# e4s2022/e4s

Measured on AMD Instinct MI355X. Metric: 1024^2 face-swap images/sec, higher is better.
Workload: dtype f32 operands as hi+lo bf16, 3 bf16 MFMAs per product, f32 accumulate (bf16x3) on the 3x3 convs whose launch fills the chip; exact f32 elsewhere; 1 GPU; E4S-core face swap at 1024^2 (2x Net3 encoder @256^2, style swap, 12 LocalMLPs, mask-guided StyleGAN2 generator K=13), BASELINE.json configs[3] shard: 8 swaps per GPU per step; per_gpu_batch=8, global_batch=8, out_size=1024, hip_graph=True, precision=as bf16x3 where the launch fills the chip (this batch), else exact fp32, parallelism=image-parallel x1

## Files before the change

### e4s_amd/csrc/conv_wino.hip

```cpp
#include "common.h"
#include <stdlib.h>
#include <type_traits>

int e4s_launch_wino1w(const e4s_conv_params& p, int ntn, int tx_n, int per_img, int ntiles, int grid, hipStream_t st);

namespace {

typedef __bf16 bf16x8 __attribute__((ext_vector_type(8)));
typedef __bf16 bf16x4 __attribute__((ext_vector_type(4)));

constexpr int NTHR = 512;
constexpr int TH = 16, TW = 16, NPAIR = TW / 2;
constexpr int VROWS = (TH + 2) * NPAIR;
constexpr int BN = 128, KC = 16, ROWB = 64;
constexpr int A_PLANE = VROWS * ROWB, A_BYTES = 4 * A_PLANE;
constexpr int B_PLANE = BN * ROWB, B_BYTES = 4 * B_PLANE;
#ifndef E4S_WINO_READS_FIRST
#define E4S_WINO_READS_FIRST 1
#endif
constexpr int WT_MIN_CHUNKS = 32;
constexpr int NITEMS = VROWS * 4;
constexpr int SMEM_WINO = 2 * A_BYTES + 2 * B_BYTES + 4 * BN * 2 * 8;

__device__ __forceinline__ int swz(int row, int g) { return row * ROWB + ((g ^ ((row >> 2) & 3)) << 4); }

__device__ __forceinline__ void split_store4(unsigned char* hi_dst, unsigned char* lo_dst, const f32x4 v) {
    const bf16x4 h = __builtin_convertvector(v, bf16x4);
    const f32x4 r = v - __builtin_convertvector(h, f32x4);
    const bf16x4 l = __builtin_convertvector(r, bf16x4);
    *reinterpret_cast<bf16x4*>(hi_dst) = h;
    *reinterpret_cast<bf16x4*>(lo_dst) = l;
}

__global__ void wino_weights_kernel(const float* __restrict__ w9, unsigned char* __restrict__ out, int Cout, int Cin) {
    const int64_t i = (int64_t)blockIdx.x * blockDim.x + threadIdx.x;
// ... 549 lines not shown
    cper = nchunk;
    if (tiles > 128 || nchunk < 4) return;
    int want = (int)((256 + tiles - 1) / tiles);
    if (want > nchunk / 2) want = nchunk / 2;
    if (want < 2) return;
    const int c = (nchunk + want - 1) / want, k = (nchunk + c - 1) / c;
    if (k < 2 || nchunk - (k - 1) * c < 2) return;
    ksplit = k;
    cper = c;
}

bool wino_covers(const e4s_conv_params& p) {
    return p.istride == 1 && p.ostride == 1 && p.ntaps == 9 && p.ncls == 1 && !p.labels && !p.rows && !p.in_scale && !p.out_scale &&
           !p.noise && p.y_cstride == 0 && p.Hi == p.Ho && p.Wi == p.Wo && p.Ha == p.Ho && p.Wa == p.Wo && p.Hi % TH == 0 &&
           p.Wi % TW == 0 && p.Cin % KC == 0 && p.Cin >= 2 * KC && p.Cout % BN == 0 && p.B > 0 &&
           (p.stats_ws == nullptr || p.stats_slots == (p.Hi / TH) * (p.Wi / TW));
}

}

extern "C" int64_t e4s_wino_weights_bytes(int Cout, int Cin) {
    if (Cout <= 0 || Cin <= 0 || Cin % KC) return -1;
    return (int64_t)3 * (Cin / KC) * 4 * Cout * ROWB * (Cout % 32 == 0 ? 2 : 1);
}

extern "C" int e4s_wino_weights_f32(const float* w9, void* out, int Cout, int Cin, void* stream) {
    if (!w9 || !out || Cout <= 0 || Cin <= 0 || Cin % KC) return (int)hipErrorInvalidValue;
    const int64_t total = (int64_t)3 * Cout * Cin;
    hipLaunchKernelGGL(wino_weights_kernel, dim3((unsigned)((total + 255) / 256)), dim3(256), 0, as_stream(stream), w9,
                       reinterpret_cast<unsigned char*>(out), Cout, Cin);
    E4S_CHECK_LAUNCH();
    return 0;
}

extern "C" int e4s_conv_wino_covers(const e4s_conv_params* p) { return p && wino_covers(*p) ? 1 : 0; }

extern "C" int64_t e4s_conv_wino_ws_floats(const e4s_conv_params* pp) {
    if (!pp || !wino_covers(*pp)) return 0;
    const e4s_conv_params& p = *pp;
    int ksplit, cper;
    wino_split(p, (int64_t)p.B * (p.Hi / TH) * (p.Wi / TW) * (p.Cout / BN), ksplit, cper);
    return ksplit > 1 ? (int64_t)ksplit * p.B * p.Ho * p.Wo * p.Cout : 0;
}

extern "C" int e4s_conv_wino_bf16x3_f32(const e4s_conv_params* pp, void* stream) {
    if (!pp) return (int)hipErrorInvalidValue;
    const e4s_conv_params& p = *pp;
    if (!p.x || !p.w || !p.y || !wino_covers(p)) return (int)hipErrorInvalidValue;
    if (p.act == 2 && !p.slope) return (int)hipErrorInvalidValue;
    const int tx_n = p.Wi / TW, per_img = (p.Hi / TH) * tx_n, ntn = p.Cout / BN;
// ... 10 lines not shown
    {
        static std::atomic<uint64_t> mv[11];
        const char* ev = getenv("E4S_WINO_VAR");
        const int var = ev ? atoi(ev) : 0;
        const void* fn = nullptr;
#define WV(V) case V: fn = (const void*)conv_wino_kernel<0, V>; if ((e = e4s_ensure_dyn_smem(fn, SMEM_WINO, mv[V]))) return e; \
              hipLaunchKernelGGL((conv_wino_kernel<0, V>), dim3((unsigned)grid), dim3(NTHR), SMEM_WINO, as_stream(stream), p, ntn, tx_n, per_img, (int)tiles, ksplit, cper); \
              E4S_CHECK_LAUNCH(); return 0;
        switch (p.in_stats ? 0 : var) {
            WV(1) WV(2) WV(3) WV(4) WV(5) WV(6) WV(7) WV(8) WV(9) WV(10)
            default: break;
        }
#undef WV
    }
#endif
    {
        const char* e1 = getenv("E4S_WINO_1W");
        const bool want = e1 ? atoi(e1) != 0 : (p.Cin / KC >= 8 && p.Cout % 32 == 0);
        if (ksplit == 1 && want) return e4s_launch_wino1w(p, ntn, tx_n, per_img, (int)tiles, (int)grid, as_stream(stream));
    }
    const char* wt_env = getenv("E4S_WINO_WT");
    const bool wt = wt_env ? atoi(wt_env) != 0 : (p.Cin / KC) / (ksplit > 0 ? ksplit : 1) >= WT_MIN_CHUNKS;
    if (wt) {
        static std::atomic<uint64_t> w0{0}, w2{0};
        if (p.in_stats) {
            if (p.Cin > 1024) return (int)hipErrorInvalidValue;
            if ((e = e4s_ensure_dyn_smem((const void*)conv_wino_kernel<2, 0, 1>, SMEM_WINO + 16384, w2))) return e;
            hipLaunchKernelGGL((conv_wino_kernel<2, 0, 1>), dim3((unsigned)grid), dim3(NTHR), SMEM_WINO + p.Cin * 16, as_stream(stream), p, ntn,
                               tx_n, per_img, (int)tiles, ksplit, cper);
        } else {
            if ((e = e4s_ensure_dyn_smem((const void*)conv_wino_kernel<0, 0, 1>, SMEM_WINO, w0))) return e;
            hipLaunchKernelGGL((conv_wino_kernel<0, 0, 1>), dim3((unsigned)grid), dim3(NTHR), SMEM_WINO, as_stream(stream), p, ntn, tx_n, per_img,
                               (int)tiles, ksplit, cper);
        }
    } else if (p.in_stats) {
// ... 14 lines not shown
```

### e4s_amd/csrc/conv_wino1w.hip

```cpp
#include "common.h"
#include <stdlib.h>
#include <type_traits>

namespace {

typedef __bf16 bf16x8 __attribute__((ext_vector_type(8)));
typedef __bf16 bf16x2 __attribute__((ext_vector_type(2)));
typedef float f32x2 __attribute__((ext_vector_type(2)));
typedef unsigned u32x2 __attribute__((ext_vector_type(2)));

constexpr int NTHR = 256;
constexpr int TH = 16, TW = 16, NPAIR = TW / 2;
constexpr int VROWS = (TH + 2) * NPAIR;
constexpr int BN = 128, KC = 16, ROWB = 64;
constexpr int A_PLANE = VROWS * ROWB, A_BYTES = 4 * A_PLANE;
constexpr int OFF_IN = 2 * A_BYTES;
constexpr int SMEM_1W = OFF_IN;
#ifndef E4S_WINO_BPF
#define E4S_WINO_BPF 1
#endif
constexpr int BPF = E4S_WINO_BPF;
static_assert(BPF == 1 || BPF == 2, "B prefetch distance");

__device__ __forceinline__ int swz(int row, int g) { return row * ROWB + ((g ^ ((row >> 2) & 3)) << 4); }

__device__ __forceinline__ void lds_barrier() {
    __builtin_amdgcn_fence(__ATOMIC_RELEASE, "workgroup", "local");
    __builtin_amdgcn_s_barrier();
    __builtin_amdgcn_fence(__ATOMIC_ACQUIRE, "workgroup", "local");
}

struct WTile {
    int n0, tb, ty0, tx0, slot;
};

struct AF { bf16x8 h[4], l[4]; };
struct BF { bf16x8 h, l; };

template <int XF>
__device__ __forceinline__ void pair_split(const float a0, const float b0, const float a1, const float b1, const float m0, const float m1,
                                           const float sg, const float r0, const float r1, unsigned& hi, unsigned& lo) {
    float v0 = __builtin_fmaf(sg, b0 - m0, a0 - m0), v1 = __builtin_fmaf(sg, b1 - m1, a1 - m1);
    if (XF == 2) {
        v0 *= r0;
        v1 *= r1;
    }
    hi = __builtin_bit_cast(unsigned, __builtin_convertvector(f32x2{v0, v1}, bf16x2));
    const float e0 = v0 - __builtin_bit_cast(float, hi << 16), e1 = v1 - __builtin_bit_cast(float, hi & 0xffff0000u);
    lo = __builtin_bit_cast(unsigned, __builtin_convertvector(f32x2{e0, e1}, bf16x2));
}

template <int XF, int VAR = 0>
__global__ __launch_bounds__(NTHR) __attribute__((amdgpu_waves_per_eu(1, 1)))
void conv_wino1w_kernel(const e4s_conv_params p, const int ntn, const int tx_n, const int per_img, const int ntiles) {
    extern __shared__ __attribute__((aligned(16))) unsigned char smem[];
    unsigned char* sA = smem;
    float* s_in = reinterpret_cast<float*>(smem + OFF_IN);

    const int tid = threadIdx.x;
    const int lane = tid & 63, wave = __builtin_amdgcn_readfirstlane(tid >> 6);
    const int li = lane & 31, kh = lane >> 5;
    const int wn = wave;
    const int G = gridDim.x;
    const int first = xcd_remap(blockIdx.x, G);
    const int mtiles = ntiles / ntn;
    const int nchunk = p.Cin / KC;
    const unsigned char* ub = reinterpret_cast<const unsigned char*>(p.w);
    auto decode = [&](int t) -> WTile {
        WTile w;
        const int nt = t / mtiles, mt = t - nt * mtiles;
        w.n0 = nt * BN;
        w.tb = mt / per_img;
        w.slot = mt - w.tb * per_img;
        const int tyb = w.slot / tx_n;
        w.ty0 = tyb * TH;
        w.tx0 = (w.slot - tyb * tx_n) * TW;
        return w;
    };

    const int cq = tid & 3;
    auto rel_of = [&](int v) -> int { return (((v >> 3) - 1) * p.Wi + 2 * (v & 7) - 1) * p.Cin + cq * 4; };
    auto flg_of = [&](int v) -> unsigned { return ((v >> 3) == 0 ? 1u : 0u) | ((v >> 3) == 17 ? 2u : 0u) | ((v & 7) == 0 ? 4u : 0u) | ((v & 7) == 7 ? 8u : 0u); };
    auto dst_of = [&](int v) -> int { return swz(v, cq >> 1) + (cq & 1) * 8; };
    const int vA = tid >> 2, vB = 64 + (tid >> 2), vQ = 128 + (lane >> 2);
    const int relA = rel_of(vA), relB = rel_of(vB), relQ = rel_of(vQ);
    const unsigned flgA = flg_of(vA), flgB = flg_of(vB), flgQ = flg_of(vQ);
    const int dstA = dst_of(vA), dstB = dst_of(vB), dstQ = dst_of(vQ) + wave * A_PLANE;
    const int qa = wave == 0 ? 0 : (wave == 2 ? 2 : 1), qb = wave == 0 ? 2 : (wave == 1 ? 2 : (wave == 2 ? 1 : 3));
    const float qsg = wave == 1 ? 1.f : -1.f;
    auto edge_of = [&](const WTile& T) -> unsigned {
        return (T.ty0 == 0 ? 1u : 0u) | (T.ty0 + TH == p.Hi ? 2u : 0u) | (T.tx0 == 0 ? 4u : 0u) | (T.tx0 + TW == p.Wi ? 8u : 0u);
    };
    auto xbase_of = [&](const WTile& T, int chunk) -> const float* {
        return p.x + (size_t)T.tb * p.Hi * p.Wi * p.Cin + ((size_t)T.ty0 * p.Wi + T.tx0) * p.Cin + chunk * KC;
    };
    auto load_px = [&](const float* xb, int rel, unsigned bad, int i, bool& ok) -> f32x4 {
        ok = !((bad & 3u) || (i == 0 && (bad & 4u)) || (i == 3 && (bad & 8u)));
        return *reinterpret_cast<const f32x4*>(xb + (ok ? rel + i * p.Cin : cq * 4));
    };
// ... 36 lines not shown
        }
        hi = __builtin_bit_cast(unsigned, __builtin_convertvector(f32x2{v[0], v[1]}, bf16x2));
        const float e0 = v[0] - __builtin_bit_cast(float, hi << 16), e1 = v[1] - __builtin_bit_cast(float, hi & 0xffff0000u);
        lo = __builtin_bit_cast(unsigned, __builtin_convertvector(f32x2{e0, e1}, bf16x2));
    };
    auto load_stats = [&](const WTile& T, int par) {
        if (XF == 2) {
            const float* st = p.in_stats + (size_t)T.tb * p.Cin * 2;
            for (int i = tid * 4; i < p.Cin * 2; i += NTHR * 4)
                *reinterpret_cast<f32x4*>(s_in + par * p.Cin * 2 + i) = *reinterpret_cast<const f32x4*>(st + i);
        }
    };

    const unsigned char* uf = ub + (size_t)3 * nchunk * 4 * p.Cout * ROWB;
    auto uf_src = [&](int ky, int chunk, int ps, int n0) -> const unsigned char* {
        return uf + ((((size_t)ky * nchunk + chunk) * 4 + ps) * (p.Cout / 32) + (n0 / 32 + wn)) * 2048 + lane * 16;
    };
    if (first >= ntiles) return;
    WTile cur = decode(first);
    int t_next = first + G;
    bool has_next = t_next < ntiles;
    WTile nxt = decode(has_next ? t_next : first);

    Item I;
    f32x4 Qa, Qb;
    bool Qoka = true, Qokb = true;
    I.okmask = 0;
    load_stats(cur, 0);
    if (XF == 2) __syncthreads();
    {
        const float* xb0 = xbase_of(cur, 0);
// ... 12 lines not shown
                item_pair(I0, mu, rs, ps, 0, h[0], l[0]);
                item_pair(I0, mu, rs, ps, 1, h[1], l[1]);
                const int a = ps * A_PLANE + dst_of(v);
                *reinterpret_cast<u32x2*>(sA + a) = u32x2{h[0], h[1]};
                *reinterpret_cast<u32x2*>(sA + (a ^ 32)) = u32x2{l[0], l[1]};
            }
        }
        const float* xb1 = xbase_of(cur, 1);
#pragma unroll
        for (int i = 0; i < 4; ++i) item_load_part(I, xb1, relA, flgA & edge, i);
        Qa = load_px(xb1, relQ, flgQ & edge, qa, Qoka);
        Qb = load_px(xb1, relQ, flgQ & edge, qb, Qokb);
    }
    __syncthreads();

    int aoff[4][3];
#pragma unroll
    for (int tm = 0; tm < 4; ++tm)
#pragma unroll
        for (int ky = 0; ky < 3; ++ky) aoff[tm][ky] = swz(tm * 32 + li + 8 * ky, kh);

    f32x16 acc[4][4];
    AF Af[2];
    BF Bf[BPF == 1 ? 1 : 3][4];
    auto ldA = [&](AF& F, const unsigned char* Abuf, int ps, int ky, int part) {
        const unsigned char* a = Abuf + ps * A_PLANE;
        const int tm = part >> 1;
        if (part & 1) F.l[tm] = *reinterpret_cast<const bf16x8*>(a + (aoff[tm][ky] ^ 32));
        else F.h[tm] = *reinterpret_cast<const bf16x8*>(a + aoff[tm][ky]);
    };
#pragma unroll
    for (int part = 0; part < 8; ++part) ldA(Af[0], sA, 0, 0, part);
#pragma unroll
    for (int ps = 0; ps < 4; ++ps) {
        const unsigned char* b = uf_src(0, 0, ps, cur.n0);
        Bf[0][ps].h = *reinterpret_cast<const bf16x8*>(b);
        Bf[0][ps].l = *reinterpret_cast<const bf16x8*>(b + 1024);
        if (BPF == 2) {
            const unsigned char* b1 = uf_src(1, 0, ps, cur.n0);
            Bf[1][ps].h = *reinterpret_cast<const bf16x8*>(b1);
            Bf[1][ps].l = *reinterpret_cast<const bf16x8*>(b1 + 1024);
        }
    }

    unsigned sg = 0, cg = 0;
    int par = 0;
    f32x4 mu = {0.f, 0.f, 0.f, 0.f}, rs = {1.f, 1.f, 1.f, 1.f};
    unsigned hh[2], ll[2];
    for (;;) {
        if (has_next) load_stats(nxt, par ^ 1);
        const unsigned edge_c = edge_of(cur), edge_n = edge_of(nxt);
#pragma unroll
        for (int ps = 0; ps < 4; ++ps)
#pragma unroll
            for (int tm = 0; tm < 4; ++tm)
#pragma unroll
                for (int r = 0; r < 16; ++r) acc[ps][tm][r] = 0.f;

        for (int chunk = 0; chunk < nchunk; ++chunk) {
            const bool in_tile = chunk + 1 < nchunk;
            const WTile& Tn = in_tile ? cur : nxt;
            const int c_n = in_tile ? chunk + 1 : 0;
            const int par_n = in_tile ? par : par ^ 1;
            const unsigned char* Ab = sA + (cg & 1) * A_BYTES;
            unsigned char* An = sA + ((cg + 1) & 1) * A_BYTES;
            const bool in2 = chunk + 2 < nchunk;
            const WTile& T2 = in2 ? cur : nxt;
            const int c_2 = in2 ? chunk + 2 : (chunk + 2 - nchunk);
            const unsigned edge_nn = in_tile ? edge_c : edge_n, edge_2 = in2 ? edge_c : edge_n;
            const float* xb_n = xbase_of(Tn, c_n);
            const float* xb_2 = xbase_of(T2, c_2);
            auto stage = [&](auto ts_c) {
                constexpr int ts = decltype(ts_c)::value;
                constexpr int ky1 = (ts + BPF) % 3;
                const int ch1 = ts + BPF < 3 ? chunk : c_n, n01 = ts + BPF < 3 ? cur.n0 : Tn.n0;
                constexpr int bs_cur = BPF == 1 ? 0 : ts, bs_ld = BPF == 1 ? 0 : (ts + 2) % 3;
#pragma unroll
                for (int ps = 0; ps < 4; ++ps) {
                    AF& Ac = Af[ps & 1];
                    AF& Ax = Af[(ps + 1) & 1];
                    const BF Bc = Bf[bs_cur][ps];
                    const unsigned char* nA = ps < 3 ? Ab : (ts < 2 ? Ab : An);
                    const int nps = (ps + 1) & 3, nky = ps < 3 ? ts : (ts + 1) % 3;
                    const unsigned char* nb = uf_src(ky1, ch1, ps, n01);
#pragma unroll
                    for (int k = 0; k < 12; ++k) {
                        const int prod = k >> 2, tm = k & 3;
                        acc[ps][tm] = prod == 0 ? __builtin_amdgcn_mfma_f32_32x32x16_bf16(Ac.h[tm], Bc.l, acc[ps][tm], 0, 0, 0)
                                    : prod == 1 ? __builtin_amdgcn_mfma_f32_32x32x16_bf16(Ac.l[tm], Bc.h, acc[ps][tm], 0, 0, 0)
                                                : __builtin_amdgcn_mfma_f32_32x32x16_bf16(Ac.h[tm], Bc.h, acc[ps][tm], 0, 0, 0);
                        if (VAR == 4) {
                            if (k == 0) Ax = Ac;
                        } else if (k < 8) ldA(Ax, nA, nps, nky, k);
                        if (VAR == 0 || VAR == 2) {
                            if (k == 8) Bf[bs_ld][ps].l = *reinterpret_cast<const bf16x8*>(nb + 1024);
                            if (k == 11) Bf[bs_ld][ps].h = *reinterpret_cast<const bf16x8*>(nb);
                        }
                        if (ps >= 2 && (VAR == 0 || VAR == 1)) {
                            const int n = (ps - 2) * 12 + k;
                            if (ts < 2 && n < 16) {
                                const int q = n >> 2, piece = n & 3;
                                if (n == 0) {
                                    stats_of(mu, rs, c_n, par_n);
                                    item_fill(I, mu);
                                }
                                if (piece == 0) item_pair(I, mu, rs, q, 0, hh[0], ll[0]);
                                if (piece == 1) item_pair(I, mu, rs, q, 1, hh[1], ll[1]);
                                const int a = q * A_PLANE + (ts == 0 ? dstA : dstB);
                                if (piece == 2) *reinterpret_cast<u32x2*>(An + a) = u32x2{hh[0], hh[1]};
                                if (piece == 3) *reinterpret_cast<u32x2*>(An + (a ^ 32)) = u32x2{ll[0], ll[1]};
                            }
                            if (ts == 0 && n >= 16 && n < 20) {
                                const f32x4 fill = XF == 2 ? mu : f32x4{0.f, 0.f, 0.f, 0.f};
                                const f32x4 da = Qoka ? Qa : fill, db = Qokb ? Qb : fill;
                                const bool nrm = XF == 2 && wave == 1;
                                if (n == 16) pair_split<XF>(da[0], db[0], da[1], db[1], nrm ? mu[0] : 0.f, nrm ? mu[1] : 0.f, qsg, rs[0], rs[1], hh[0], ll[0]);
                                if (n == 17) pair_split<XF>(da[2], db[2], da[3], db[3], nrm ? mu[2] : 0.f, nrm ? mu[3] : 0.f, qsg, rs[2], rs[3], hh[1], ll[1]);
                                if (n == 18) *reinterpret_cast<u32x2*>(An + dstQ) = u32x2{hh[0], hh[1]};
                                if (n == 19) *reinterpret_cast<u32x2*>(An + (dstQ ^ 32)) = u32x2{ll[0], ll[1]};
                            }
                            if (ts == 0 && n >= 20) item_load_part(I, xb_n, relB, flgB & edge_nn, n - 20);
                            if (ts == 2 && n >= 16 && n < 20) item_load_part(I, xb_2, relA, flgA & edge_2, n - 16);
                            if (ts == 2 && n == 20) Qa = load_px(xb_2, relQ, flgQ & edge_2, qa, Qoka);
                            if (ts == 2 && n == 21) Qb = load_px(xb_2, relQ, flgQ & edge_2, qb, Qokb);
                        }
                        __builtin_amdgcn_sched_barrier(0);
                    }
                    if (ps == 1 && VAR != 4) {
                        lds_barrier();
                        __builtin_amdgcn_sched_barrier(0);
                    }
                }
                ++sg;
            };
            stage(std::integral_constant<int, 0>{});
            stage(std::integral_constant<int, 1>{});
            stage(std::integral_constant<int, 2>{});
            ++cg;
        }

        {
            const float gain = (p.act == 1) ? p.gain : 1.f;
            const bool do_act = p.act != 0;
            const bool stats = p.stats_ws != nullptr;
            float* yb = p.y + (size_t)cur.tb * p.Ho * p.Wo * p.Cout;
            const int co = cur.n0 + wn * 32 + li;
            const float bsv = p.bias ? p.bias[co] : 0.f;
            const float slp = (p.act == 2) ? p.slope[co] : p.alpha;
            double st_s = 0.0, st_q = 0.0;
#pragma unroll
            for (int tm = 0; tm < 4; ++tm) {
#pragma unroll
                for (int g = 0; g < 4; ++g) {
                    float y0[4], y1[4];
#pragma unroll
                    for (int i = 0; i < 4; ++i) {
                        const int r = 4 * g + i;
                        const float m0 = acc[0][tm][r], m1 = acc[1][tm][r], m2 = acc[2][tm][r], m3 = acc[3][tm][r];
                        float a = (m0 + m1) + m2 + bsv;
                        float b = (m1 - m2) - m3 + bsv;
                        if (do_act) {
                            a = (a > 0.f ? a : a * slp) * gain;
                            b = (b > 0.f ? b : b * slp) * gain;
                        }
                        y0[i] = a;
                        y1[i] = b;
                        if (stats) {
                            st_s += (double)a + (double)b;
                            st_q += (double)a * (double)a + (double)b * (double)b;
                        }
                    }
                    quad_transpose4(y0[0], y0[1], y0[2], y0[3], li);
                    quad_transpose4(y1[0], y1[1], y1[2], y1[3], li);
// ... 11 lines not shown
                    double* slot = p.stats_ws + (((size_t)cur.tb * p.Cout + co) * p.stats_slots + cur.slot) * 2;
                    slot[0] = st_s;
                    slot[1] = st_q;
                }
            }
        }
        if (!has_next) break;
        cur = nxt;
        par ^= 1;
        t_next += G;
        has_next = t_next < ntiles;
        if (has_next) nxt = decode(t_next);
    }
}

}

int e4s_launch_wino1w(const e4s_conv_params& p, int ntn, int tx_n, int per_img, int ntiles, int grid, hipStream_t st) {
    static std::atomic<uint64_t> m0{0}, m2{0};
    int e;
#ifdef E4S_ABLATIONS
    {
        const char* ev = getenv("E4S_WINO_1W_VAR");
        const int var = ev ? atoi(ev) : 0;
        const void* fn = nullptr;
#define WV(V) case V: fn = (const void*)conv_wino1w_kernel<0, V>; if ((e = (int)hipFuncSetAttribute(fn, hipFuncAttributeMaxDynamicSharedMemorySize, SMEM_1W))) return e; \
              hipLaunchKernelGGL((conv_wino1w_kernel<0, V>), dim3((unsigned)grid), dim3(NTHR), SMEM_1W, st, p, ntn, tx_n, per_img, ntiles); \
              E4S_CHECK_LAUNCH(); return 0;
        switch (p.in_stats ? 0 : var) {
            WV(1) WV(2) WV(3) WV(4)
            default: break;
        }
#undef WV
    }
#endif
    if (p.in_stats) {
        if (p.Cin > 1024) return (int)hipErrorInvalidValue;
        if ((e = e4s_ensure_dyn_smem((const void*)conv_wino1w_kernel<2>, SMEM_1W + 16384, m2))) return e;
        hipLaunchKernelGGL(conv_wino1w_kernel<2>, dim3((unsigned)grid), dim3(NTHR), SMEM_1W + p.Cin * 16, st, p, ntn, tx_n, per_img, ntiles);
    } else {
        if ((e = e4s_ensure_dyn_smem((const void*)conv_wino1w_kernel<0>, SMEM_1W, m0))) return e;
        hipLaunchKernelGGL(conv_wino1w_kernel<0>, dim3((unsigned)grid), dim3(NTHR), SMEM_1W, st, p, ntn, tx_n, per_img, ntiles);
    }
    E4S_CHECK_LAUNCH();
    return 0;
}
```

### e4s_amd/csrc/ops.hip

```cpp
#include "common.h"

namespace {

__device__ __forceinline__ float bias_act_one(float x, float ref, int code, float alpha, float scale) {
    float y;
    switch (code) {
        case 12: case 32: y = 0.f; break;
        case 30: y = (x > 0.f) ? x : x * alpha; break;
        case 31: y = (ref > 0.f) ? x : x * alpha; break;
        default: y = x; break;
    }
    return y * scale;
}

__global__ void fused_bias_act_v4(const f32x4* __restrict__ x, const float* __restrict__ b,
                                  const f32x4* __restrict__ ref, f32x4* __restrict__ y, int64_t n4,
                                  int step_b, int size_b, int code, float alpha, float scale) {
    const int64_t stride = (int64_t)gridDim.x * blockDim.x;
    for (int64_t i = (int64_t)blockIdx.x * blockDim.x + threadIdx.x; i < n4; i += stride) {
        f32x4 v = x[i];
        if (b) {
            const float bv = b[((i * 4) / step_b) % size_b];
            v += bv;
        }
// ... 75 lines not shown
        if (oy >= out_h || ox >= out_w) continue;
        const int my = oy * down_y - pad_y0, mx = ox * down_x - pad_x0;
        const int iy_first = floordiv(my + up_y - 1, up_y), ix_first = floordiv(mx + up_x - 1, up_x);
        float acc = 0.f;
        for (int iy = iy_first, jy = iy_first * up_y - my; jy < kh; ++iy, jy += up_y) {
            const float* row = sx + (iy - in_y0) * tin_w;
            for (int ix = ix_first, jx = ix_first * up_x - mx; jx < kw; ++ix, jx += up_x)
                acc += row[ix - in_x0] * sk[jy * kw + jx];
        }
        y[(((int64_t)mj * out_h + oy) * out_w + ox) * minor + mi] = acc;
    }
}

}

extern "C" int e4s_abi_version(void) { return 15; }
extern "C" const char* e4s_build_arch(void) { return "gfx950"; }

extern "C" int e4s_fused_bias_act_f32(const float* x, const float* b, const float* ref, float* y, int64_t n,
                                      int step_b, int size_b, int act, int grad, float alpha, float scale,
                                      void* stream) {
    if (n <= 0) return 0;
    const int code = act * 10 + grad;
    if (code == 31 && !ref) return (int)hipErrorInvalidValue;
    if (b && (step_b <= 0 || size_b <= 0)) return (int)hipErrorInvalidValue;
    const bool vec = (n % 4 == 0) && (!b || step_b % 4 == 0) &&
                     ((reinterpret_cast<uintptr_t>(x) | reinterpret_cast<uintptr_t>(y) |
                       reinterpret_cast<uintptr_t>(ref)) % 16 == 0);
    const int block = 256;
    if (vec) {
        const int64_t n4 = n / 4;
// ... 135 lines not shown
```

### e4s_amd/kernels.py

```python
import contextlib
import ctypes
import math
import os
import threading

import torch

from . import lib
from .lib import ConvBwdParams, ConvParams, ConvWgradParams, c_p, call, fptr, ptr, stream

BM = 128
PRECISION = os.environ.get("E4S_PRECISION", "auto")
if PRECISION not in ("f32", "bf16x3", "auto"):
    raise RuntimeError(f"E4S_PRECISION must be f32, bf16x3 or auto, got {PRECISION!r}")
BF16X3_MIN_BLOCKS = int(os.environ.get("E4S_BF16X3_MIN_BLOCKS", "128"))
LRELU_GAIN = math.sqrt(2.0)


def _f32(t):
    if t.dtype != torch.float32:
        raise RuntimeError(f"expected float32 tensor, got {t.dtype}")
    return t.contiguous()


# ... 376 lines not shown

def split16_bf16x2(w, out=None):
    w = _f32(w)
    out = _into(out, split16_shape(w.shape), w.device)
    cout, cin = w.shape[-2], w.shape[-1]
    rows = w.numel() // (cout * cin)
    if lib.load().e4s_split16_bytes(rows, cout, cin) != out.numel() * 4:
        raise RuntimeError("split16_bf16x2: buffer size")
    call("e4s_split16_bf16x2_f32", fptr(w), ptr(out), rows, cout, cin, stream())
    return out


REGION_1W = os.environ.get("E4S_REGION_1W", "1") != "0"
LAST_REGION_PATH = 0
WINO = os.environ.get("E4S_WINO", "1") == "1"


def wino_eligible(b, h, w, cin, cout, in_stats=False):
    if not WINO or PRECISION == "f32":
        return False
    if h % 16 or w % 16 or cin % 16 or cin < 32 or cout % 128:
        return False
    if in_stats and cin > 1024:
        return False
    if PRECISION == "bf16x3":
        return True
    tiles = b * (h // 16) * (w // 16) * (cout // 128)
    if tiles >= BF16X3_MIN_BLOCKS:
        return True
    nchunk = cin // 16
# ... 19 lines not shown
    y = torch.empty(b, h, w, cout, device=x.device, dtype=torch.float32)
    p = ConvParams()
    p.x, p.w, p.y = fptr(x), ptr(u), fptr(y)
    p.rows = p.tiles = p.meta = None
    p.B, p.Ha, p.Wa, p.Hi, p.Wi, p.Ho, p.Wo, p.Cin, p.Cout = b, h, w, h, w, h, w, cin, cout
    p.istride, p.ostride, p.ntaps, p.ncls, p.groups_per_batch = 1, 1, 9, 1, 1
    p.bias, p.slope = fptr(bias), fptr(slope)
    p.act, p.alpha, p.gain = act, alpha, gain
    p.in_stats = fptr(in_stats)
    fused = None
    if want_stats and act != 0:
        raise RuntimeError("conv_wino: output statistics are those of the raw conv output (act = 0)")
    nws = lib.load().e4s_conv_wino_ws_floats(ctypes.byref(p))
    skws = torch.empty(nws, device=x.device, dtype=torch.float32) if nws else None
    p.splitk_ws = fptr(skws)
    if want_stats and not nws:
        slots = (h // 16) * (w // 16)
        fused = torch.empty(b * cout * slots * 2, device=x.device, dtype=torch.float64)
        p.stats_ws, p.stats_slots = ptr(fused), slots
    call("e4s_conv_wino_bf16x3_f32", ctypes.byref(p), stream())
    if fused is None:
        if not want_stats:
            return y
        stats, pooled = instnorm_stats(y, want_pooled=True)
        return y, (stats, se_gate(pooled, se[0], se[1]) if se is not None else pooled)
    stats = torch.empty(b, cout, 2, device=x.device, dtype=torch.float32)
    pooled = torch.empty(b, cout, device=x.device, dtype=torch.float32)
    if se is not None:
        call("e4s_instnorm_finalize_se_f32", ptr(fused), fptr(stats), fptr(se[0]), fptr(se[1]), fptr(pooled), b, h * w, cout,
             se[0].shape[0], p.stats_slots, 1e-5, stream())
    else:
        call("e4s_instnorm_finalize_f32", ptr(fused), fptr(stats), fptr(pooled), b, h * w, cout, p.stats_slots, 1e-5, stream())
# ... 898 lines not shown
```

### e4s_amd/lib.py

```python
import ctypes
import os

import torch

_HERE = os.path.dirname(os.path.abspath(__file__))
LIB_PATH = os.environ.get("E4S_LIB_PATH") or os.path.join(_HERE, "libe4s_hip.so")
ABI_VERSION = 15

c_p = ctypes.c_void_p
c_i = ctypes.c_int
c_l = ctypes.c_int64
c_f = ctypes.c_float
c_d = ctypes.c_double


STYLE_GRAD_MAX_JOBS = 32


class StyleGradJob(ctypes.Structure):
    _fields_ = [
        ("ds_raw", c_p), ("dd_d", c_p), ("d", c_p), ("s", c_p), ("wsq", c_p), ("dws", c_p), ("w3", c_p), ("wmod", c_p), ("ds_total", c_p),
        ("conv_scale", c_f), ("mod_scale", c_f), ("G", c_i), ("Cin", c_i), ("Cout", c_i), ("slot", c_i), ("masked", c_i),
    ]

# ... 91 lines not shown
    "e4s_torgb_finish_f32": [c_p, c_p, c_p, c_p, c_p, c_i, c_i, c_i, c_p],
    "e4s_rowdot_multi_f32": [c_p, c_i, c_p, c_p, c_i, c_i, c_i, c_p],
    "e4s_ema_f32": [c_p, c_p, c_l, c_d, c_p],
    "e4s_adam_step_dev_f32": [c_p, c_p, c_p, c_p, c_l, c_d, c_p, c_d, c_d, c_d, c_d, c_p, c_p],
    "e4s_advance_i64": [c_p, c_l, c_p],
    "e4s_conv_smallcin_col2im_f32": [c_p, c_p] + [c_i] * 10 + [c_p],
    "e4s_region_scale_f32": [c_p, c_p, c_p, c_i, c_i, c_i, c_p, c_i, c_i, c_i, c_i, c_i, c_p],
    "e4s_col2im_region_nsplit": [c_i, c_i, c_i, c_i],
    "e4s_col2im_region_f32": [c_p, c_p, c_p, c_p, c_i, c_i, c_i, c_p, c_p, c_p, c_i, c_i, c_i, c_i, c_i, c_p],
    "e4s_act_bwd_demod_nsplit": [c_i, c_i, c_i, c_i],
    "e4s_act_bwd_demod_f32": [c_p, c_p, c_p, c_p, c_p, c_l, c_p, c_f, c_f, c_p, c_i, c_i, c_i, c_p, c_p, c_i, c_i, c_i, c_i, c_p],
    "e4s_pixel_unshuffle2_f32": [c_p, c_p, c_i, c_i, c_i, c_i, c_p],
    "e4s_wino_weights_bytes": [c_i, c_i],
    "e4s_wino_weights_f32": [c_p, c_p, c_i, c_i, c_p],
    "e4s_conv_wino_covers": [c_p],
    "e4s_conv_wino_ws_floats": [c_p],
    "e4s_conv_wino_bf16x3_f32": [c_p, c_p],
    "e4s_adam_multi_dev_f32": [c_i, c_p, c_p, c_p, c_p, c_p, c_p, c_d, c_p, c_d, c_d, c_d, c_d, c_p],
    "e4s_ema_multi_f32": [c_i, c_p, c_p, c_p, c_d, c_p],
    "e4s_torgb_bwd_x_f32": [c_p, c_p, c_p, c_i, c_i, c_i, c_p, c_i, c_i, c_i, c_i, c_i, c_p],
    "e4s_shift_scale_f32": [c_p, c_p, c_p, c_i, c_i, c_i, c_p] + [c_i] * 12 + [c_p],
    "e4s_torgb_f32": [c_p, c_p, c_p, c_p, c_p, c_p, c_i, c_i, c_i, c_p, c_i, c_i, c_i, c_i, c_p],
    "e4s_mask_mul_add_f32": [c_p, c_p, c_p] + [c_i] * 10 + [c_p],
    "e4s_noise_bias_act_nhwc_f32": [c_p, c_p, c_p, c_l, c_p, c_p, c_i, c_i, c_i, c_f, c_f, c_p],
    "e4s_nchw_to_nhwc_f32": [c_p, c_p, c_i, c_i, c_i, c_i, c_p],
    "e4s_nhwc_to_nchw_f32": [c_p, c_p, c_i, c_i, c_i, c_i, c_p],
    "e4s_const_input_f32": [c_p, c_p, c_i, c_i, c_i, c_i, c_p],
    "e4s_resize_bilinear_f32": [c_p, c_p] + [c_i] * 6 + [c_p],
    "e4s_conv3x3_small_f32": [c_p, c_p, c_p] + [c_i] * 5 + [c_p],
    "e4s_conv3x3_stem_f32": [c_p, c_p, c_p, c_p] + [c_i] * 5 + [c_p],
# ... 112 lines not shown
```

### include/e4s_hip.h

```cpp
#ifndef E4S_HIP_H
#define E4S_HIP_H
#include <stdint.h>

#ifdef __cplusplus
extern "C" {
#endif

int e4s_abi_version(void);
const char* e4s_build_arch(void);


int e4s_fused_bias_act_f32(const float* x, const float* b, const float* ref, float* y, int64_t n,
                           int step_b, int size_b, int act, int grad, float alpha, float scale,
                           void* stream);

int e4s_upfirdn2d_f32(const float* x, const float* k, float* y, int major, int in_h, int in_w, int minor,
                      int kh, int kw, int up_x, int up_y, int down_x, int down_y,
                      int pad_x0, int pad_x1, int pad_y0, int pad_y1, void* stream);

int e4s_channel_sum_f32(const float* g, float* out, int64_t n, int step_b, int size_b, void* stream);


int e4s_rowdot_f32(const float* in, int64_t in_stride, const float* M, const float* bias, float* out,
                   int G, int O, int K, int mode, float scale, void* stream);
// ... 189 lines not shown
int64_t e4s_colsum_ws_floats(int64_t rows, int C);
int e4s_scale_dot_f32(float* u, const float* x, const float* s, float* ds, float* ws, int B, int64_t hw, int C, void* stream);
int64_t e4s_scale_dot_ws_floats(int B, int64_t hw, int C);
int e4s_adam_step_f32(float* p, const float* grad, float* m, float* v, int64_t n, double lr, double beta1, double beta2,
                      double eps, double weight_decay, int step, void* stream);
int e4s_adam_step_dev_f32(float* p, const float* grad, float* m, float* v, int64_t n, double lr, const double* lr_dev, double beta1,
                          double beta2, double eps, double weight_decay, const int64_t* step, void* stream);
int e4s_advance_i64(int64_t* steps, int64_t n, void* stream);
int e4s_adam_multi_dev_f32(int count, float* const* p, const float* const* grad, float* const* m, float* const* v, const int64_t* n,
                           const int64_t* const* step, double lr, const double* lr_dev, double beta1, double beta2, double eps,
                           double weight_decay, void* stream);
int e4s_ema_multi_f32(int count, float* const* dst, const float* const* src, const int64_t* n, double decay, void* stream);
int64_t e4s_wino_weights_bytes(int Cout, int Cin);
int e4s_wino_weights_f32(const float* w9, void* out, int Cout, int Cin, void* stream);
int e4s_conv_wino_covers(const e4s_conv_params* p);
int64_t e4s_conv_wino_ws_floats(const e4s_conv_params* p);
int e4s_conv_wino_bf16x3_f32(const e4s_conv_params* p, void* stream);
int e4s_subpixel_weights_f32(const float* w, void* out, int Cout, int Cin, void* stream);
int e4s_upconv_bf16x3_f32(const e4s_conv_params* p, const float* k4, void* stream);

int e4s_conv_c32_bf16x3_f32(const e4s_conv_params* p, const float* rgb_ws, float* rgb_partial, void* stream);
int e4s_torgb_finish_f32(const float* partial, const float* bias, const float* skip, const float* k4, float* out, int B, int H,
                         int W, void* stream);

int e4s_mask_to_u8(const float* mask, uint8_t* out, int B, int H, int W, int Hm, int Wm, void* stream);
int e4s_erode_u8(const uint8_t* src, uint8_t* dst, int B, int H, int W, int radius, int border_value, void* stream);
int e4s_gaussian_blur_u8(const uint8_t* src, uint8_t* dst, int B, int H, int W, int ksize, const int* taps_fixed8, void* stream);
int e4s_alpha_composite_u8(const uint8_t* face, const uint8_t* target, const uint8_t* alpha, uint8_t* out, int B, int H, int W,
                           void* stream);
int e4s_pyrdown_u8(const uint8_t* src, uint8_t* dst, int B, int H, int W, int C, void* stream);
// ... 94 lines not shown
```

Baseline: 491.2 images/s.

## Add wide-N 8x16 tile variant to single-wave Winograd bf16x3 conv kernel

Templates the single-wave Winograd conv kernel on a tile shape. When Cout is a multiple of 256 (the default), the new variant uses 8-row spatial tiles with 256 output channels per block, so each wave holds two 32-column B fragments and two A row-tiles instead of one B and four A. This shifts reuse from the A operand toward the weights and changes how B loads are scheduled, and adds a stats-slot layout tied to the tile height, which the Python side now queries. Risks include higher register pressure from two B fragments, fewer tiles per image when filling the GPU, and weight prefetch being disabled for the wide path (BP=1).

```diff
diff --git a/e4s_amd/csrc/conv_wino.hip b/e4s_amd/csrc/conv_wino.hip
--- a/e4s_amd/csrc/conv_wino.hip
+++ b/e4s_amd/csrc/conv_wino.hip
@@ -2,7 +2,7 @@
 #include <stdlib.h>
 #include <type_traits>
 
-int e4s_launch_wino1w(const e4s_conv_params& p, int ntn, int tx_n, int per_img, int ntiles, int grid, hipStream_t st);
+int e4s_launch_wino1w(const e4s_conv_params& p, int wide, int ntn, int tx_n, int per_img, int ntiles, int grid, hipStream_t st);
 
 namespace {
 
@@ -19,6 +19,7 @@
 #define E4S_WINO_READS_FIRST 1
 #endif
 constexpr int WT_MIN_CHUNKS = 32;
+constexpr int TH_WIDE = 8, BN_WIDE = 256;
 constexpr int NITEMS = VROWS * 4;
 constexpr int SMEM_WINO = 2 * A_BYTES + 2 * B_BYTES + 4 * BN * 2 * 8;
 
@@ -598,7 +599,18 @@
     return p.istride == 1 && p.ostride == 1 && p.ntaps == 9 && p.ncls == 1 && !p.labels && !p.rows && !p.in_scale && !p.out_scale &&
            !p.noise && p.y_cstride == 0 && p.Hi == p.Ho && p.Wi == p.Wo && p.Ha == p.Ho && p.Wa == p.Wo && p.Hi % TH == 0 &&
            p.Wi % TW == 0 && p.Cin % KC == 0 && p.Cin >= 2 * KC && p.Cout % BN == 0 && p.B > 0 &&
-           (p.stats_ws == nullptr || p.stats_slots == (p.Hi / TH) * (p.Wi / TW));
+           (p.stats_ws == nullptr || p.stats_slots == (p.Hi / TH) * (p.Wi / TW) ||
+            (p.Cout % BN_WIDE == 0 && p.stats_slots == (p.Hi / TH_WIDE) * (p.Wi / TW)));
+}
+
+int wino_path(const e4s_conv_params& p, int ksplit) {
+    const char* e1 = getenv("E4S_WINO_1W");
+    const bool want = e1 ? atoi(e1) != 0 : (p.Cin / KC >= 8 && p.Cout % 32 == 0);
+    if (ksplit != 1 || !want) return 1;
+    if (p.Cout % BN_WIDE) return 2;
+    const char* et = getenv("E4S_WINO_1W_TILE");
+    const bool wide = et ? atoi(et) != 0 : true;
+    return wide ? 3 : 2;
 }
 
 }
@@ -618,6 +630,13 @@
 }
 
 extern "C" int e4s_conv_wino_covers(const e4s_conv_params* p) { return p && wino_covers(*p) ? 1 : 0; }
+
+extern "C" int e4s_conv_wino_path(const e4s_conv_params* pp) {
+    if (!pp || !wino_covers(*pp)) return 0;
+    int ksplit, cper;
+    wino_split(*pp, (int64_t)pp->B * (pp->Hi / TH) * (pp->Wi / TW) * (pp->Cout / BN), ksplit, cper);
+    return wino_path(*pp, ksplit);
+}
 
 extern "C" int64_t e4s_conv_wino_ws_floats(const e4s_conv_params* pp) {
     if (!pp || !wino_covers(*pp)) return 0;
@@ -658,11 +677,14 @@
 #undef WV
     }
 #endif
-    {
-        const char* e1 = getenv("E4S_WINO_1W");
-        const bool want = e1 ? atoi(e1) != 0 : (p.Cin / KC >= 8 && p.Cout % 32 == 0);
-        if (ksplit == 1 && want) return e4s_launch_wino1w(p, ntn, tx_n, per_img, (int)tiles, (int)grid, as_stream(stream));
+    const int path = wino_path(p, ksplit);
+    if (path >= 2) {
+        const bool wide = path == 3;
+        const int pi = wide ? (p.Hi / TH_WIDE) * tx_n : per_img;
+        if (p.stats_ws && p.stats_slots != pi) return (int)hipErrorInvalidValue;
+        return e4s_launch_wino1w(p, wide ? 1 : 0, wide ? p.Cout / BN_WIDE : ntn, tx_n, pi, (int)tiles, (int)grid, as_stream(stream));
     }
+    if (p.stats_ws && p.stats_slots != per_img) return (int)hipErrorInvalidValue;
     const char* wt_env = getenv("E4S_WINO_WT");
     const bool wt = wt_env ? atoi(wt_env) != 0 : (p.Cin / KC) / (ksplit > 0 ? ksplit : 1) >= WT_MIN_CHUNKS;
     if (wt) {
diff --git a/e4s_amd/csrc/conv_wino1w.hip b/e4s_amd/csrc/conv_wino1w.hip
--- a/e4s_amd/csrc/conv_wino1w.hip
+++ b/e4s_amd/csrc/conv_wino1w.hip
@@ -10,12 +10,19 @@
 typedef unsigned u32x2 __attribute__((ext_vector_type(2)));
 
 constexpr int NTHR = 256;
-constexpr int TH = 16, TW = 16, NPAIR = TW / 2;
-constexpr int VROWS = (TH + 2) * NPAIR;
-constexpr int BN = 128, KC = 16, ROWB = 64;
-constexpr int A_PLANE = VROWS * ROWB, A_BYTES = 4 * A_PLANE;
-constexpr int OFF_IN = 2 * A_BYTES;
-constexpr int SMEM_1W = OFF_IN;
+constexpr int TW = 16, NPAIR = TW / 2;
+constexpr int KC = 16, ROWB = 64;
+template <int W>
+struct Tile {
+    static constexpr int TH = W ? 8 : 16;
+    static constexpr int VROWS = (TH + 2) * NPAIR;
+    static constexpr int NTM = TH / 4, NCB = W ? 2 : 1;
+    static constexpr int BN = 4 * 32 * NCB;
+    static constexpr int A_PLANE = VROWS * ROWB, A_BYTES = 4 * A_PLANE;
+    static constexpr int VQ0 = VROWS - 16;
+    static constexpr int OFF_IN = 2 * A_BYTES;
+    static constexpr int SMEM = OFF_IN;
+};
 #ifndef E4S_WINO_BPF
 #define E4S_WINO_BPF 1
 #endif
@@ -34,8 +41,10 @@
     int n0, tb, ty0, tx0, slot;
 };
 
-struct AF { bf16x8 h[4], l[4]; };
-struct BF { bf16x8 h, l; };
+template <int NTM>
+struct AFt { bf16x8 h[NTM], l[NTM]; };
+template <int NCB>
+struct BFt { bf16x8 h[NCB], l[NCB]; };
 
 template <int XF>
 __device__ __forceinline__ void pair_split(const float a0, const float b0, const float a1, const float b1, const float m0, const float m1,
@@ -50,12 +59,17 @@
     lo = __builtin_bit_cast(unsigned, __builtin_convertvector(f32x2{e0, e1}, bf16x2));
 }
 
-template <int XF, int VAR = 0>
+template <int XF, int VAR = 0, int W = 0>
 __global__ __launch_bounds__(NTHR) __attribute__((amdgpu_waves_per_eu(1, 1)))
 void conv_wino1w_kernel(const e4s_conv_params p, const int ntn, const int tx_n, const int per_img, const int ntiles) {
+    using C = Tile<W>;
+    constexpr int TH = C::TH, VROWS = C::VROWS, BN = C::BN, A_PLANE = C::A_PLANE, A_BYTES = C::A_BYTES, NTM = C::NTM, NCB = C::NCB;
+    constexpr int BP = W ? 1 : BPF;
+    using AF = AFt<NTM>;
+    using BF = BFt<NCB>;
     extern __shared__ __attribute__((aligned(16))) unsigned char smem[];
     unsigned char* sA = smem;
-    float* s_in = reinterpret_cast<float*>(smem + OFF_IN);
+    float* s_in = reinterpret_cast<float*>(smem + C::OFF_IN);
 
     const int tid = threadIdx.x;
     const int lane = tid & 63, wave = __builtin_amdgcn_readfirstlane(tid >> 6);
@@ -80,9 +94,9 @@
 
     const int cq = tid & 3;
     auto rel_of = [&](int v) -> int { return (((v >> 3) - 1) * p.Wi + 2 * (v & 7) - 1) * p.Cin + cq * 4; };
-    auto flg_of = [&](int v) -> unsigned { return ((v >> 3) == 0 ? 1u : 0u) | ((v >> 3) == 17 ? 2u : 0u) | ((v & 7) == 0 ? 4u : 0u) | ((v & 7) == 7 ? 8u : 0u); };
+    auto flg_of = [&](int v) -> unsigned { return ((v >> 3) == 0 ? 1u : 0u) | ((v >> 3) == TH + 1 ? 2u : 0u) | ((v & 7) == 0 ? 4u : 0u) | ((v & 7) == 7 ? 8u : 0u); };
     auto dst_of = [&](int v) -> int { return swz(v, cq >> 1) + (cq & 1) * 8; };
-    const int vA = tid >> 2, vB = 64 + (tid >> 2), vQ = 128 + (lane >> 2);
+    const int vA = tid >> 2, vB = 64 + (tid >> 2), vQ = C::VQ0 + (lane >> 2);
     const int relA = rel_of(vA), relB = rel_of(vB), relQ = rel_of(vQ);
     const unsigned flgA = flg_of(vA), flgB = flg_of(vB), flgQ = flg_of(vQ);
     const int dstA = dst_of(vA), dstB = dst_of(vB), dstQ = dst_of(vQ) + wave * A_PLANE;
@@ -149,7 +163,12 @@
 
     const unsigned char* uf = ub + (size_t)3 * nchunk * 4 * p.Cout * ROWB;
     auto uf_src = [&](int ky, int chunk, int ps, int n0) -> const unsigned char* {
-        return uf + ((((size_t)ky * nchunk + chunk) * 4 + ps) * (p.Cout / 32) + (n0 / 32 + wn)) * 2048 + lane * 16;
+        return uf + ((((size_t)ky * nchunk + chunk) * 4 + ps) * (p.Cout / 32) + (n0 / 32 + wn * NCB)) * 2048 + lane * 16;
+    };
+    auto ldB = [&](BF& F, const unsigned char* b, int part) {
+        const int cb = part >> 1;
+        if (part & 1) F.l[cb] = *reinterpret_cast<const bf16x8*>(b + cb * 2048 + 1024);
+        else F.h[cb] = *reinterpret_cast<const bf16x8*>(b + cb * 2048);
     };
     if (first >= ntiles) return;
     WTile cur = decode(first);
@@ -192,15 +211,15 @@
     }
     __syncthreads();
 
-    int aoff[4][3];
-#pragma unroll
-    for (int tm = 0; tm < 4; ++tm)
+    int aoff[NTM][3];
+#pragma unroll
+    for (int tm = 0; tm < NTM; ++tm)
 #pragma unroll
         for (int ky = 0; ky < 3; ++ky) aoff[tm][ky] = swz(tm * 32 + li + 8 * ky, kh);
 
-    f32x16 acc[4][4];
+    f32x16 acc[4][NCB][NTM];
     AF Af[2];
-    BF Bf[BPF == 1 ? 1 : 3][4];
+    BF Bf[BP == 1 ? 1 : 3][4];
     auto ldA = [&](AF& F, const unsigned char* Abuf, int ps, int ky, int part) {
         const unsigned char* a = Abuf + ps * A_PLANE;
         const int tm = part >> 1;
@@ -208,16 +227,13 @@
         else F.h[tm] = *reinterpret_cast<const bf16x8*>(a + aoff[tm][ky]);
     };
 #pragma unroll
-    for (int part = 0; part < 8; ++part) ldA(Af[0], sA, 0, 0, part);
+    for (int part = 0; part < 2 * NTM; ++part) ldA(Af[0], sA, 0, 0, part);
 #pragma unroll
     for (int ps = 0; ps < 4; ++ps) {
-        const unsigned char* b = uf_src(0, 0, ps, cur.n0);
-        Bf[0][ps].h = *reinterpret_cast<const bf16x8*>(b);
-        Bf[0][ps].l = *reinterpret_cast<const bf16x8*>(b + 1024);
-        if (BPF == 2) {
-            const unsigned char* b1 = uf_src(1, 0, ps, cur.n0);
-            Bf[1][ps].h = *reinterpret_cast<const bf16x8*>(b1);
-            Bf[1][ps].l = *reinterpret_cast<const bf16x8*>(b1 + 1024);
+#pragma unroll
+        for (int part = 0; part < 2 * NCB; ++part) {
+            ldB(Bf[0][ps], uf_src(0, 0, ps, cur.n0), part);
+            if (BP == 2) ldB(Bf[1][ps], uf_src(1, 0, ps, cur.n0), part);
         }
     }
 
@@ -231,9 +247,11 @@
 #pragma unroll
         for (int ps = 0; ps < 4; ++ps)
 #pragma unroll
-            for (int tm = 0; tm < 4; ++tm)
-#pragma unroll
-                for (int r = 0; r < 16; ++r) acc[ps][tm][r] = 0.f;
+            for (int cb = 0; cb < NCB; ++cb)
+#pragma unroll
+                for (int tm = 0; tm < NTM; ++tm)
+#pragma unroll
+                    for (int r = 0; r < 16; ++r) acc[ps][cb][tm][r] = 0.f;
 
         for (int chunk = 0; chunk < nchunk; ++chunk) {
             const bool in_tile = chunk + 1 < nchunk;
@@ -250,9 +268,9 @@
             const float* xb_2 = xbase_of(T2, c_2);
             auto stage = [&](auto ts_c) {
                 constexpr int ts = decltype(ts_c)::value;
-                constexpr int ky1 = (ts + BPF) % 3;
-                const int ch1 = ts + BPF < 3 ? chunk : c_n, n01 = ts + BPF < 3 ? cur.n0 : Tn.n0;
-                constexpr int bs_cur = BPF == 1 ? 0 : ts, bs_ld = BPF == 1 ? 0 : (ts + 2) % 3;
+                constexpr int ky1 = (ts + BP) % 3;
+                const int ch1 = ts + BP < 3 ? chunk : c_n, n01 = ts + BP < 3 ? cur.n0 : Tn.n0;
+                constexpr int bs_cur = BP == 1 ? 0 : ts, bs_ld = BP == 1 ? 0 : (ts + 2) % 3;
 #pragma unroll
                 for (int ps = 0; ps < 4; ++ps) {
                     AF& Ac = Af[ps & 1];
@@ -263,20 +281,27 @@
                     const unsigned char* nb = uf_src(ky1, ch1, ps, n01);
 #pragma unroll
                     for (int k = 0; k < 12; ++k) {
-                        const int prod = k >> 2, tm = k & 3;
-                        acc[ps][tm] = prod == 0 ? __builtin_amdgcn_mfma_f32_32x32x16_bf16(Ac.h[tm], Bc.l, acc[ps][tm], 0, 0, 0)
-                                    : prod == 1 ? __builtin_amdgcn_mfma_f32_32x32x16_bf16(Ac.l[tm], Bc.h, acc[ps][tm], 0, 0, 0)
-                                                : __builtin_amdgcn_mfma_f32_32x32x16_bf16(Ac.h[tm], Bc.h, acc[ps][tm], 0, 0, 0);
+                        const int prod = k >> 2, tm = W ? (k & 1) : (k & 3), cb = W ? ((k >> 1) & 1) : 0;
+                        acc[ps][cb][tm] = prod == 0 ? __builtin_amdgcn_mfma_f32_32x32x16_bf16(Ac.h[tm], Bc.l[cb], acc[ps][cb][tm], 0, 0, 0)
+                                        : prod == 1 ? __builtin_amdgcn_mfma_f32_32x32x16_bf16(Ac.l[tm], Bc.h[cb], acc[ps][cb][tm], 0, 0, 0)
+                                                    : __builtin_amdgcn_mfma_f32_32x32x16_bf16(Ac.h[tm], Bc.h[cb], acc[ps][cb][tm], 0, 0, 0);
                         if (VAR == 4) {
                             if (k == 0) Ax = Ac;
-                        } else if (k < 8) ldA(Ax, nA, nps, nky, k);
+                        } else if (k < 2 * NTM) ldA(Ax, nA, nps, nky, k);
                         if (VAR == 0 || VAR == 2) {
-                            if (k == 8) Bf[bs_ld][ps].l = *reinterpret_cast<const bf16x8*>(nb + 1024);
-                            if (k == 11) Bf[bs_ld][ps].h = *reinterpret_cast<const bf16x8*>(nb);
+                            if (W) {
+                                if (k == 4) ldB(Bf[bs_ld][ps], nb, 1);
+                                if (k == 5) ldB(Bf[bs_ld][ps], nb, 3);
+                                if (k == 10) ldB(Bf[bs_ld][ps], nb, 0);
+                                if (k == 11) ldB(Bf[bs_ld][ps], nb, 2);
+                            } else {
+                                if (k == 8) ldB(Bf[bs_ld][ps], nb, 1);
+                                if (k == 11) ldB(Bf[bs_ld][ps], nb, 0);
+                            }
                         }
                         if (ps >= 2 && (VAR == 0 || VAR == 1)) {
                             const int n = (ps - 2) * 12 + k;
-                            if (ts < 2 && n < 16) {
+                            if (ts < (W ? 1 : 2) && n < 16) {
                                 const int q = n >> 2, piece = n & 3;
                                 if (n == 0) {
                                     stats_of(mu, rs, c_n, par_n);
@@ -297,7 +322,7 @@
                                 if (n == 18) *reinterpret_cast<u32x2*>(An + dstQ) = u32x2{hh[0], hh[1]};
                                 if (n == 19) *reinterpret_cast<u32x2*>(An + (dstQ ^ 32)) = u32x2{ll[0], ll[1]};
                             }
-                            if (ts == 0 && n >= 20) item_load_part(I, xb_n, relB, flgB & edge_nn, n - 20);
+                            if (!W && ts == 0 && n >= 20) item_load_part(I, xb_n, relB, flgB & edge_nn, n - 20);
                             if (ts == 2 && n >= 16 && n < 20) item_load_part(I, xb_2, relA, flgA & edge_2, n - 16);
                             if (ts == 2 && n == 20) Qa = load_px(xb_2, relQ, flgQ & edge_2, qa, Qoka);
                             if (ts == 2 && n == 21) Qb = load_px(xb_2, relQ, flgQ & edge_2, qb, Qokb);
@@ -317,24 +342,25 @@
             ++cg;
         }
 
-        {
+#pragma unroll
+        for (int cb = 0; cb < NCB; ++cb) {
             const float gain = (p.act == 1) ? p.gain : 1.f;
             const bool do_act = p.act != 0;
             const bool stats = p.stats_ws != nullptr;
             float* yb = p.y + (size_t)cur.tb * p.Ho * p.Wo * p.Cout;
-            const int co = cur.n0 + wn * 32 + li;
+            const int co = cur.n0 + (wn * NCB + cb) * 32 + li;
             const float bsv = p.bias ? p.bias[co] : 0.f;
             const float slp = (p.act == 2) ? p.slope[co] : p.alpha;
             double st_s = 0.0, st_q = 0.0;
 #pragma unroll
-            for (int tm = 0; tm < 4; ++tm) {
+            for (int tm = 0; tm < NTM; ++tm) {
 #pragma unroll
                 for (int g = 0; g < 4; ++g) {
                     float y0[4], y1[4];
 #pragma unroll
                     for (int i = 0; i < 4; ++i) {
                         const int r = 4 * g + i;
-                        const float m0 = acc[0][tm][r], m1 = acc[1][tm][r], m2 = acc[2][tm][r], m3 = acc[3][tm][r];
+                        const float m0 = acc[0][cb][tm][r], m1 = acc[1][cb][tm][r], m2 = acc[2][cb][tm][r], m3 = acc[3][cb][tm][r];
                         float a = (m0 + m1) + m2 + bsv;
                         float b = (m1 - m2) - m3 + bsv;
                         if (do_act) {
@@ -376,19 +402,26 @@
     }
 }
 
-}
-
-int e4s_launch_wino1w(const e4s_conv_params& p, int ntn, int tx_n, int per_img, int ntiles, int grid, hipStream_t st) {
-    static std::atomic<uint64_t> m0{0}, m2{0};
+template <int XF, int VAR, int W>
+int launch_1w(const e4s_conv_params& p, int ntn, int tx_n, int per_img, int ntiles, int grid, hipStream_t st) {
+    static std::atomic<uint64_t> done{0};
+    const int stat_bytes = XF == 2 ? p.Cin * 16 : 0;
     int e;
+    if ((e = e4s_ensure_dyn_smem((const void*)conv_wino1w_kernel<XF, VAR, W>, Tile<W>::SMEM + (XF == 2 ? 16384 : 0), done))) return e;
+    hipLaunchKernelGGL((conv_wino1w_kernel<XF, VAR, W>), dim3((unsigned)grid), dim3(NTHR), Tile<W>::SMEM + stat_bytes, st, p, ntn, tx_n, per_img, ntiles);
+    E4S_CHECK_LAUNCH();
+    return 0;
+}
+
+}
+
+int e4s_launch_wino1w(const e4s_conv_params& p, int wide, int ntn, int tx_n, int per_img, int ntiles, int grid, hipStream_t st) {
+    if (wide && p.Cout % Tile<1>::BN) return (int)hipErrorInvalidValue;
 #ifdef E4S_ABLATIONS
     {
         const char* ev = getenv("E4S_WINO_1W_VAR");
         const int var = ev ? atoi(ev) : 0;
-        const void* fn = nullptr;
-#define WV(V) case V: fn = (const void*)conv_wino1w_kernel<0, V>; if ((e = (int)hipFuncSetAttribute(fn, hipFuncAttributeMaxDynamicSharedMemorySize, SMEM_1W))) return e; \
-              hipLaunchKernelGGL((conv_wino1w_kernel<0, V>), dim3((unsigned)grid), dim3(NTHR), SMEM_1W, st, p, ntn, tx_n, per_img, ntiles); \
-              E4S_CHECK_LAUNCH(); return 0;
+#define WV(V) case V: return wide ? launch_1w<0, V, 1>(p, ntn, tx_n, per_img, ntiles, grid, st) : launch_1w<0, V, 0>(p, ntn, tx_n, per_img, ntiles, grid, st);
         switch (p.in_stats ? 0 : var) {
             WV(1) WV(2) WV(3) WV(4)
             default: break;
@@ -398,12 +431,7 @@
 #endif
     if (p.in_stats) {
         if (p.Cin > 1024) return (int)hipErrorInvalidValue;
-        if ((e = e4s_ensure_dyn_smem((const void*)conv_wino1w_kernel<2>, SMEM_1W + 16384, m2))) return e;
-        hipLaunchKernelGGL(conv_wino1w_kernel<2>, dim3((unsigned)grid), dim3(NTHR), SMEM_1W + p.Cin * 16, st, p, ntn, tx_n, per_img, ntiles);
-    } else {
-        if ((e = e4s_ensure_dyn_smem((const void*)conv_wino1w_kernel<0>, SMEM_1W, m0))) return e;
-        hipLaunchKernelGGL(conv_wino1w_kernel<0>, dim3((unsigned)grid), dim3(NTHR), SMEM_1W, st, p, ntn, tx_n, per_img, ntiles);
-    }
-    E4S_CHECK_LAUNCH();
-    return 0;
-}
+        return wide ? launch_1w<2, 0, 1>(p, ntn, tx_n, per_img, ntiles, grid, st) : launch_1w<2, 0, 0>(p, ntn, tx_n, per_img, ntiles, grid, st);
+    }
+    return wide ? launch_1w<0, 0, 1>(p, ntn, tx_n, per_img, ntiles, grid, st) : launch_1w<0, 0, 0>(p, ntn, tx_n, per_img, ntiles, grid, st);
+}
diff --git a/e4s_amd/csrc/ops.hip b/e4s_amd/csrc/ops.hip
--- a/e4s_amd/csrc/ops.hip
+++ b/e4s_amd/csrc/ops.hip
@@ -113,7 +113,7 @@
 
 }
 
-extern "C" int e4s_abi_version(void) { return 15; }
+extern "C" int e4s_abi_version(void) { return 16; }
 extern "C" const char* e4s_build_arch(void) { return "gfx950"; }
 
 extern "C" int e4s_fused_bias_act_f32(const float* x, const float* b, const float* ref, float* y, int64_t n,
diff --git a/e4s_amd/kernels.py b/e4s_amd/kernels.py
--- a/e4s_amd/kernels.py
+++ b/e4s_amd/kernels.py
@@ -414,6 +414,7 @@
 REGION_1W = os.environ.get("E4S_REGION_1W", "1") != "0"
 LAST_REGION_PATH = 0
 WINO = os.environ.get("E4S_WINO", "1") == "1"
+LAST_WINO_PATH = 0
 
 
 def wino_eligible(b, h, w, cin, cout, in_stats=False):
@@ -463,8 +464,10 @@
     nws = lib.load().e4s_conv_wino_ws_floats(ctypes.byref(p))
     skws = torch.empty(nws, device=x.device, dtype=torch.float32) if nws else None
     p.splitk_ws = fptr(skws)
+    global LAST_WINO_PATH
+    LAST_WINO_PATH = lib.load().e4s_conv_wino_path(ctypes.byref(p))
     if want_stats and not nws:
-        slots = (h // 16) * (w // 16)
+        slots = (h // (8 if LAST_WINO_PATH == 3 else 16)) * (w // 16)
         fused = torch.empty(b * cout * slots * 2, device=x.device, dtype=torch.float64)
         p.stats_ws, p.stats_slots = ptr(fused), slots
     call("e4s_conv_wino_bf16x3_f32", ctypes.byref(p), stream())
diff --git a/e4s_amd/lib.py b/e4s_amd/lib.py
--- a/e4s_amd/lib.py
+++ b/e4s_amd/lib.py
@@ -5,7 +5,7 @@
 
 _HERE = os.path.dirname(os.path.abspath(__file__))
 LIB_PATH = os.environ.get("E4S_LIB_PATH") or os.path.join(_HERE, "libe4s_hip.so")
-ABI_VERSION = 15
+ABI_VERSION = 16
 
 c_p = ctypes.c_void_p
 c_i = ctypes.c_int
@@ -129,6 +129,7 @@
     "e4s_wino_weights_bytes": [c_i, c_i],
     "e4s_wino_weights_f32": [c_p, c_p, c_i, c_i, c_p],
     "e4s_conv_wino_covers": [c_p],
+    "e4s_conv_wino_path": [c_p],
     "e4s_conv_wino_ws_floats": [c_p],
     "e4s_conv_wino_bf16x3_f32": [c_p, c_p],
     "e4s_adam_multi_dev_f32": [c_i, c_p, c_p, c_p, c_p, c_p, c_p, c_d, c_p, c_d, c_d, c_d, c_d, c_p],
diff --git a/include/e4s_hip.h b/include/e4s_hip.h
--- a/include/e4s_hip.h
+++ b/include/e4s_hip.h
@@ -227,6 +227,7 @@
 int64_t e4s_wino_weights_bytes(int Cout, int Cin);
 int e4s_wino_weights_f32(const float* w9, void* out, int Cout, int Cin, void* stream);
 int e4s_conv_wino_covers(const e4s_conv_params* p);
+int e4s_conv_wino_path(const e4s_conv_params* p);
 int64_t e4s_conv_wino_ws_floats(const e4s_conv_params* p);
 int e4s_conv_wino_bf16x3_f32(const e4s_conv_params* p, void* stream);
 int e4s_subpixel_weights_f32(const float* w, void* out, int Cout, int Cin, void* stream);
```

New measurement: 489.5 images/s, median of 2. About the same (-0.3%).
